# kahrendt/microWakeWord

Measured on NVIDIA H100. Metric: streams_x_frames_per_sec, higher is better.
Workload: dtype f32

## Files before the change

microwakeword_b200/csrc/mww_common.h:

```cpp
#pragma once

#include <stdint.h>

#if defined(__CUDACC__)
#define MWW_HD __host__ __device__ __forceinline__
#define MWW_D __device__ __forceinline__
#else
#define MWW_HD inline
#define MWW_D inline
#endif

namespace mww {

constexpr int kNumChannels = 40;
constexpr int kWindow = 480;
constexpr int kHop = 160;
constexpr int kFftSize = 512;
constexpr int kNcfft = 256;
constexpr float kFeatureScale = 0.0390625f;

MWW_HD int msb32(uint32_t x) {
#if defined(__CUDA_ARCH__)
    return 32 - __clz((int)x);
#else
    return x ? 32 - __builtin_clz(x) : 0;
#endif
}

MWW_HD int32_t sext16(int32_t v) { return (int32_t)(int16_t)v; }

MWW_HD uint32_t pack16(int32_t lo, int32_t hi) { return ((uint32_t)lo & 0xFFFFu) | ((uint32_t)hi << 16); }
MWW_HD int32_t unpack_lo(uint32_t w) { return (int32_t)(int16_t)(w & 0xFFFFu); }
MWW_HD int32_t unpack_hi(uint32_t w) { return ((int32_t)w) >> 16; }

MWW_HD int32_t max3i(int32_t a, int32_t b, int32_t c) { const int32_t m = a > b ? a : b; return m > c ? m : c; }
MWW_HD int32_t min3i(int32_t a, int32_t b, int32_t c) { const int32_t m = a < b ? a : b; return m < c ? m : c; }

MWW_HD int64_t mad_wide_s32(int32_t a, int32_t b, int64_t c) { return (int64_t)a * (int64_t)b + c; }

}
```

microwakeword_b200/csrc/mww_frontend.cu:

```cuda
#include <cuda_runtime.h>
#include <stdlib.h>

#include "mww_frontend_dev.cuh"
#include "mww_kernels.h"

namespace mww {

__device__ __forceinline__ void cp_async16(void *smem_dst, const void *gmem_src) {
    const unsigned dst = (unsigned)__cvta_generic_to_shared(smem_dst);
    asm volatile("cp.async.cg.shared.global [%0], [%1], 16;" ::"r"(dst), "l"(gmem_src));
}
__device__ __forceinline__ void cp_async_commit_and_wait_all() {
    asm volatile("cp.async.commit_group;\ncp.async.wait_group 0;" ::: "memory");
}

__device__ __forceinline__ void stage8(int16_t *dst, const int16_t *src) { cp_async16(dst, src); }
__device__ __forceinline__ void stage8(int16_t *dst, const float *src) {
    const float4 a = reinterpret_cast<const float4 *>(src)[0], b = reinterpret_cast<const float4 *>(src)[1];
    *reinterpret_cast<uint4 *>(dst) = make_uint4(pack16(pcm16_from_f32(a.x), pcm16_from_f32(a.y)), pack16(pcm16_from_f32(a.z), pcm16_from_f32(a.w)),
                                                 pack16(pcm16_from_f32(b.x), pcm16_from_f32(b.y)), pack16(pcm16_from_f32(b.z), pcm16_from_f32(b.w)));
}

template <typename T>
__device__ __forceinline__ void k1_load_audio_async(int tid, K1Smem &sm, int buf, const int16_t *carry, int used,
                                                    const T *audio, int n_samples, int f0) {
    const int base = kHop * f0;
    for (int v = tid; v < kGroupSamples / 8; v += kK1Threads) {
        const int vi = base + 8 * v;
        int16_t *dst = &sm.audio[buf][8 * v];
        if (vi < used) cp_async16(dst, carry + vi);
        else if (vi - used < n_samples) stage8(dst, audio + (vi - used));
        else *reinterpret_cast<uint4 *>(dst) = make_uint4(0, 0, 0, 0);
    }
}

template <typename T>
__device__ __forceinline__ void k1_packed_load_audio_async(int tid, K1Smem &sm, const int16_t *carry, int used, const T *audio,
                                                           long long audio_stride, int n_samples, long long s0, int n_streams, int spc, int fps) {
    const int span8 = (fps + 2) * (kHop / 8), used8 = used / 8, n8 = n_samples / 8;
    int16_t *dst0 = &sm.audio[0][0];
    for (int i = tid; i < spc * span8; i += kK1Threads) {
        const int sl = i / span8, v8 = i - sl * span8;
        int16_t *dst = dst0 + 8 * i;
        const long long s = s0 + sl;
        if (s < n_streams && v8 < used8) cp_async16(dst, carry + s * kWindow + 8 * v8);
        else if (s < n_streams && v8 - used8 < n8) stage8(dst, audio + s * audio_stride + 8 * (v8 - used8));
        else *reinterpret_cast<uint4 *>(dst) = make_uint4(0, 0, 0, 0);
    }
}

template <bool kFuseK2, int kOcc, typename T>
__global__ void __launch_bounds__(kK1Threads, kOcc)
k1_spectral_kernel(FrontendParams P, const int16_t *__restrict__ carry, int used,
                   const T *__restrict__ audio, long long audio_stride, int n_samples, int n_frames,
                   int groups_per_block, int vec_ok, uint32_t *__restrict__ vout, uint32_t *__restrict__ estimate,
                   uint16_t *__restrict__ feat, long long feat_stream_stride) {
    extern __shared__ __align__(16) unsigned char k1_smem_raw[];
    K1Smem &sm = *reinterpret_cast<K1Smem *>(k1_smem_raw);
    const int tid = threadIdx.x;
    const long long s = blockIdx.x;
    K1Lane lane;
    if (kOcc <= 3) k1_lane_init(tid, P, lane);
    else k1_stage_lane_twiddles(tid, sm, P);
    const K1LaneShared lane_sh{&sm.lane_tw[tid & 15][0]};
    k1_stage_tables(tid, sm, P);

    const int n_groups = (n_frames + kFramesPerGroup - 1) / kFramesPerGroup;
    const int g_begin = blockIdx.y * groups_per_block;
    const int g_end = min(g_begin + groups_per_block, n_groups);
    const int16_t *my_carry = carry + s * kWindow;
    const T *my_audio = audio + s * audio_stride;
    uint32_t est = 0;
    if (kFuseK2 && tid < kNumChannels) est = estimate[s * kNumChannels + tid];
    if (g_begin < g_end) {
        if (vec_ok) k1_load_audio_async(tid, sm, 0, my_carry, used, my_audio, n_samples, g_begin * kFramesPerGroup);
        else k1_load_audio(tid, sm, 0, my_carry, used, my_audio, n_samples, g_begin * kFramesPerGroup);
    }
    for (int g = g_begin; g < g_end; ++g) {
        const int buf = (g - g_begin) & 1;
        cp_async_commit_and_wait_all();
        __syncthreads();
        if (g + 1 < g_end) {
            if (vec_ok) k1_load_audio_async(tid, sm, buf ^ 1, my_carry, used, my_audio, n_samples, (g + 1) * kFramesPerGroup);
            else k1_load_audio(tid, sm, buf ^ 1, my_carry, used, my_audio, n_samples, (g + 1) * kFramesPerGroup);
        }
        const int f0 = g * kFramesPerGroup;
        K1Pass1Ctx ctx;
        k1_window_fft1<2>(tid, sm, buf, (kHop / 2) * (tid >> 4), P, ctx);
        __syncthreads();
        if (kOcc <= 3) k1_fft_pass2(tid, sm, lane); else k1_fft_pass2(tid, sm, lane_sh);
        __syncthreads();
        k1_real_energy(tid, sm, P);
        __syncthreads();
        const int f = f0 + (tid >> 4);
        if (!kFuseK2) {
            k1_filterbank(tid, sm, P, f < n_frames ? vout + (s * n_frames + f) * kNumChannels : nullptr);
        } else {
            k1_filterbank(tid, sm, P, &sm.A[tid >> 4][0]);
            __syncthreads();
            const int n_valid = min(kFramesPerGroup, n_frames - f0);
            if (tid < kNumChannels) k2_group_chain(tid, sm, n_valid, est);
            __syncthreads();
            k2_group_outputs(tid, sm, n_valid, feat + s * feat_stream_stride + (long long)f0 * kNumChannels);
        }
    }
    if (kFuseK2 && tid < kNumChannels) estimate[s * kNumChannels + tid] = est;
}

template <typename T>
__global__ void __launch_bounds__(kK1Threads, 3)
k1_spectral_hop_kernel(FrontendParams P, const int16_t *__restrict__ carry, int used, const T *__restrict__ audio,
                       long long audio_stride, int n_samples, int n_frames, int hop, uint32_t *__restrict__ estimate,
                       uint16_t *__restrict__ feat, long long feat_stream_stride) {
    extern __shared__ __align__(16) unsigned char k1_smem_raw[];
    K1Smem &sm = *reinterpret_cast<K1Smem *>(k1_smem_raw);
    const int tid = threadIdx.x;
    const long long s = blockIdx.x;
    K1Lane lane;
    k1_lane_init(tid, P, lane);
    k1_stage_tables(tid, sm, P);
    const int fpg = k1_hop_frames_per_group(hop);
    const int n_groups = (n_frames + fpg - 1) / fpg;
    const int16_t *my_carry = carry + s * kWindow;
    const T *my_audio = audio + s * audio_stride;
    uint32_t est = 0;
    if (tid < kNumChannels) est = estimate[s * kNumChannels + tid];
    for (int g = 0; g < n_groups; ++g) {
        const int f0 = g * fpg;
        __syncthreads();
        k1_hop_load_audio(tid, sm, my_carry, used, my_audio, n_samples, hop * f0, (fpg - 1) * hop + kWindow);
        __syncthreads();
        K1Pass1Ctx ctx;
        k1_window_fft1<2>(tid, sm, 0, k1_hop_pair_base(tid >> 4, hop, fpg), P, ctx);
        __syncthreads();
        k1_fft_pass2(tid, sm, lane);
        __syncthreads();
        k1_real_energy(tid, sm, P);
        __syncthreads();
        k1_filterbank(tid, sm, P, &sm.A[tid >> 4][0]);
        __syncthreads();
        const int n_valid = min(fpg, n_frames - f0);
        if (tid < kNumChannels) k2_group_chain(tid, sm, n_valid, est);
        __syncthreads();
        k2_group_outputs(tid, sm, n_valid, feat + s * feat_stream_stride + (long long)f0 * kNumChannels);
    }
    if (tid < kNumChannels) estimate[s * kNumChannels + tid] = est;
}

template <typename T>
__global__ void __launch_bounds__(kK1Threads, 3)
k1_spectral_packed_kernel(FrontendParams P, const int16_t *__restrict__ carry, int used,
                          const T *__restrict__ audio, long long audio_stride, int n_samples, int n_streams, int fps, int spc,
                          int vec_ok, uint32_t *__restrict__ vout) {
    extern __shared__ __align__(16) unsigned char k1_smem_raw[];
    K1Smem &sm = *reinterpret_cast<K1Smem *>(k1_smem_raw);
    const int tid = threadIdx.x;
    const long long s0 = (long long)blockIdx.x * spc;
    K1Lane lane;
    k1_lane_init(tid, P, lane);
    k1_stage_tables(tid, sm, P);
    if (vec_ok) {
        k1_packed_load_audio_async(tid, sm, carry, used, audio, audio_stride, n_samples, s0, n_streams, spc, fps);
        cp_async_commit_and_wait_all();
    } else {
        k1_packed_load_audio(tid, sm, carry, used, audio, audio_stride, n_samples, s0, n_streams, spc, fps);
    }
    __syncthreads();
    const int fl = tid >> 4;
    K1Pass1Ctx ctx;
    k1_window_fft1<2>(tid, sm, 0, k1_packed_pair_base(fl < spc * fps ? fl : 0, fps), P, ctx);
    __syncthreads();
    k1_fft_pass2(tid, sm, lane);
    __syncthreads();
    k1_real_energy(tid, sm, P);
    __syncthreads();
    const long long s = s0 + fl / fps;
    const bool active = fl < spc * fps && s < n_streams;
    k1_filterbank(tid, sm, P, active ? vout + (s * fps + fl % fps) * kNumChannels : nullptr);
}

template <typename T>
__global__ void __launch_bounds__(kK1Threads, 3)
k1k2_packed_kernel(FrontendParams P, int16_t *__restrict__ carry, int used, const T *__restrict__ audio,
                   long long audio_stride, int n_samples, int n_streams, int fps, int spc, int vec_ok, uint32_t *__restrict__ estimate,
                   uint16_t *__restrict__ feat, long long feat_stream_stride, int new_used) {
    extern __shared__ __align__(16) unsigned char k1_smem_raw[];
    K1Smem &sm = *reinterpret_cast<K1Smem *>(k1_smem_raw);
    const int tid = threadIdx.x;
    const long long s0 = (long long)blockIdx.x * spc;
    K1Lane lane;
    k1_lane_init(tid, P, lane);
    k1_stage_tables(tid, sm, P);
    if (vec_ok) {
        k1_packed_load_audio_async(tid, sm, carry, used, audio, audio_stride, n_samples, s0, n_streams, spc, fps);
        cp_async_commit_and_wait_all();
    } else {
        k1_packed_load_audio(tid, sm, carry, used, audio, audio_stride, n_samples, s0, n_streams, spc, fps);
    }
    __syncthreads();
    const int fl = tid >> 4;
    K1Pass1Ctx ctx;
    k1_window_fft1<2>(tid, sm, 0, k1_packed_pair_base(fl < spc * fps ? fl : 0, fps), P, ctx);
    __syncthreads();
    k1_fft_pass2(tid, sm, lane);
    __syncthreads();
    k1_real_energy(tid, sm, P);
    __syncthreads();
    k1_filterbank(tid, sm, P, fl < spc * fps ? &sm.A[fl][0] : nullptr);
    __syncthreads();
    for (int t = tid; t < spc * kNumChannels; t += kK1Threads) {
        const int sl = t / kNumChannels, ch = t - sl * kNumChannels;
        const long long s = s0 + sl;
        if (s < n_streams) {
            const uint32_t smoothing = (ch & 1) ? kOddSmoothing : kEvenSmoothing;
            uint32_t est = estimate[s * kNumChannels + ch];
            uint16_t *out = feat + s * feat_stream_stride + ch;
            for (int f = 0; f < fps; ++f) out[(long long)f * kNumChannels] = k2_channel_step(sm.A[sl * fps + f][ch], est, smoothing, sm.gain_lut, sm.log_lut);
            estimate[s * kNumChannels + ch] = est;
        }
    }
    const int span = (fps + 2) * kHop, consumed = fps * kHop;
    const int16_t *staged = &sm.audio[0][0];
    if (vec_ok) {
        for (int i = tid; i < spc * (kWindow / 8); i += kK1Threads) {
            const int sl = i / (kWindow / 8), v8 = i - sl * (kWindow / 8);
            if (s0 + sl >= n_streams) continue;
            uint4 v = make_uint4(0, 0, 0, 0);
            if (8 * v8 < new_used) v = *reinterpret_cast<const uint4 *>(staged + sl * span + consumed + 8 * v8);
            *reinterpret_cast<uint4 *>(carry + (s0 + sl) * kWindow + 8 * v8) = v;
        }
    } else {
        for (int i = tid; i < spc * kWindow; i += kK1Threads) {
            const int sl = i / kWindow, k = i - sl * kWindow;
            if (s0 + sl >= n_streams) continue;
            carry[(s0 + sl) * kWindow + k] = k < new_used ? staged[sl * span + consumed + k] : (int16_t)0;
        }
    }
}

__global__ void __launch_bounds__(256)
k2_temporal_kernel(FrontendParams P, const uint32_t *__restrict__ vin, int n_streams, int n_frames,
                   uint32_t *__restrict__ estimate, uint16_t *__restrict__ feat, long long feat_stream_stride) {
    __shared__ int16_t gain_lut[128];
    __shared__ uint16_t log_lut[132];
    for (int i = threadIdx.x; i < 128; i += blockDim.x) gain_lut[i] = P.gain_lut[i];
    for (int i = threadIdx.x; i < 132; i += blockDim.x) log_lut[i] = P.log_lut[i];
    __syncthreads();
    const long long idx = (long long)blockIdx.x * blockDim.x + threadIdx.x;
    if (idx >= (long long)n_streams * kNumChannels) return;
    const long long s = idx / kNumChannels;
    const int ch = (int)(idx - s * kNumChannels);
    const uint32_t smoothing = (ch & 1) ? kOddSmoothing : kEvenSmoothing;
    uint32_t est = estimate[idx];
    const uint32_t *v = vin + s * (long long)n_frames * kNumChannels + ch;
    uint16_t *out = feat + s * feat_stream_stride + ch;
    int f = 0;
    for (; f + 4 <= n_frames; f += 4) {
        uint32_t x[4];
#pragma unroll
        for (int q = 0; q < 4; ++q) x[q] = __ldcs(v + (long long)(f + q) * kNumChannels);
#pragma unroll
        for (int q = 0; q < 4; ++q) out[(long long)(f + q) * kNumChannels] = k2_channel_step(x[q], est, smoothing, gain_lut, log_lut);
    }
    for (; f < n_frames; ++f) out[(long long)f * kNumChannels] = k2_channel_step(v[(long long)f * kNumChannels], est, smoothing, gain_lut, log_lut);
    estimate[idx] = est;
}

template <typename T>
__global__ void __launch_bounds__(128)
carry_update_kernel(int16_t *__restrict__ carry, int used, const T *__restrict__ audio, long long audio_stride,
                    int n_samples, int consumed, int new_used) {
    const long long s = blockIdx.x;
    int16_t *c = carry + s * kWindow;
    const T *a = audio + s * audio_stride;
    int16_t tmp[4];
#pragma unroll
    for (int q = 0; q < 4; ++q) {
        const int i = threadIdx.x + 128 * q;
        int16_t val = 0;
        if (i < new_used) {
            const int vi = consumed + i;
            val = vi < used ? c[vi] : pcm16(a[vi - used]);
        }
        tmp[q] = val;
    }
    __syncthreads();
#pragma unroll
    for (int q = 0; q < 4; ++q) {
        const int i = threadIdx.x + 128 * q;
        if (i < kWindow) c[i] = tmp[q];
    }
}


namespace {
template <typename K>
cudaError_t k1_opt_in(K kernel, bool (&done)[64]) {
    if (!first_launch_on_this_device(done)) return cudaSuccess;
    return cudaFuncSetAttribute(kernel, cudaFuncAttributeMaxDynamicSharedMemorySize, kK1SmemBytes);
}
template <typename T>
int audio_vec_ok(const int16_t *carry, int used, const T *audio, long long audio_stride, int n_samples) {
    return (used % 8 == 0) && (n_samples % 8 == 0) && (audio_stride % 8 == 0) &&
           (reinterpret_cast<uintptr_t>(audio) % 16 == 0) && (reinterpret_cast<uintptr_t>(carry) % 16 == 0);
}
}

bool frontend_clip_fuses(int n_streams, int n_frames, int sm_count) {
    return n_frames > 8 && (long long)n_streams >= (long long)sm_count * 3 * 4;
}

template <typename T>
cudaError_t launch_k1(const FrontendParams &P, const int16_t *carry, int used, const T *audio,
                      long long audio_stride, int n_samples, int n_streams, int n_frames, uint32_t *vout, int sm_count,
                      cudaStream_t st) {
    if (n_frames <= 0 || n_streams <= 0) return cudaSuccess;
    const int vec_ok = audio_vec_ok(carry, used, audio, audio_stride, n_samples);
    if (n_frames <= 8 && n_streams >= 2) {
        static bool done[64] = {};
        cudaError_t e = k1_opt_in(k1_spectral_packed_kernel<T>, done);
        if (e != cudaSuccess) return e;
        const int spc = k1_packed_streams(n_frames);
        const unsigned grid = (unsigned)((n_streams + spc - 1) / spc);
        k1_spectral_packed_kernel<T><<<grid, kK1Threads, kK1SmemBytes, st>>>(P, carry, used, audio, audio_stride, n_samples, n_streams, n_frames, spc, vec_ok, vout);
        return cudaGetLastError();
    }
    static bool done[64] = {};
    cudaError_t e = k1_opt_in(k1_spectral_kernel<false, 3, T>, done);
    if (e != cudaSuccess) return e;
    const int n_groups = (n_frames + kFramesPerGroup - 1) / kFramesPerGroup;
    int chunks = 1;
    const long long want = (long long)sm_count * 3 * 4;
    if (n_streams < want) chunks = (int)min((long long)n_groups, (want + n_streams - 1) / n_streams);
    const int gpb = (n_groups + chunks - 1) / chunks;
    chunks = (n_groups + gpb - 1) / gpb;
    dim3 grid((unsigned)n_streams, (unsigned)chunks);
    k1_spectral_kernel<false, 3, T><<<grid, kK1Threads, kK1SmemBytes, st>>>(P, carry, used, audio, audio_stride, n_samples, n_frames, gpb, vec_ok, vout,
                                                                         nullptr, nullptr, 0);
    return cudaGetLastError();
}

template <typename T>
cudaError_t launch_frontend_clip_fused(const FrontendParams &P, const int16_t *carry, int used, const T *audio, long long audio_stride,
                                       int n_samples, int n_streams, int n_frames, uint32_t *estimate, uint16_t *feat, long long feat_stream_stride,
                                       cudaStream_t st) {
    if (n_frames <= 0 || n_streams <= 0) return cudaSuccess;
    static bool done3[64] = {}, done4[64] = {};
    static const int occ = getenv("MWW_K1_OCC") ? atoi(getenv("MWW_K1_OCC")) : 4;
    cudaError_t e = occ == 3 ? k1_opt_in(k1_spectral_kernel<true, 3, T>, done3) : k1_opt_in(k1_spectral_kernel<true, 4, T>, done4);
    if (e != cudaSuccess) return e;
    const int vec_ok = audio_vec_ok(carry, used, audio, audio_stride, n_samples);
    const int n_groups = (n_frames + kFramesPerGroup - 1) / kFramesPerGroup;
    dim3 grid((unsigned)n_streams, 1u);
    if (occ == 3)
        k1_spectral_kernel<true, 3, T><<<grid, kK1Threads, kK1SmemBytes, st>>>(P, carry, used, audio, audio_stride, n_samples, n_frames, n_groups, vec_ok,
                                                                               nullptr, estimate, feat, feat_stream_stride);
    else
        k1_spectral_kernel<true, 4, T><<<grid, kK1Threads, kK1SmemBytes, st>>>(P, carry, used, audio, audio_stride, n_samples, n_frames, n_groups, vec_ok,
                                                                               nullptr, estimate, feat, feat_stream_stride);
    return cudaGetLastError();
}

template <typename T>
cudaError_t launch_frontend_hop(const FrontendParams &P, const int16_t *carry, int used, const T *audio, long long audio_stride,
                                int n_samples, int n_streams, int n_frames, int hop, uint32_t *estimate, uint16_t *feat,
                                long long feat_stream_stride, cudaStream_t st) {
    if (n_frames <= 0 || n_streams <= 0) return cudaSuccess;
    static bool done[64] = {};
    cudaError_t e = k1_opt_in(k1_spectral_hop_kernel<T>, done);
    if (e != cudaSuccess) return e;
    k1_spectral_hop_kernel<T><<<(unsigned)n_streams, kK1Threads, kK1SmemBytes, st>>>(P, carry, used, audio, audio_stride, n_samples, n_frames, hop,
                                                                                    estimate, feat, feat_stream_stride);
    return cudaGetLastError();
}

bool frontend_fusable(int used, int n_samples, int n_frames) {
    const int new_used = used + n_samples - n_frames * kHop;
    return n_frames >= 1 && n_frames <= 8 && new_used >= 0 && new_used <= 2 * kHop;
}

template <typename T>
cudaError_t launch_frontend_fused(const FrontendParams &P, int16_t *carry, int used, const T *audio,
                                  long long audio_stride, int n_samples, int n_streams, int n_frames, uint32_t *estimate, uint16_t *feat,
                                  long long feat_stream_stride, cudaStream_t st) {
    if (n_streams <= 0) return cudaSuccess;
    static bool done[64] = {};
    cudaError_t e = k1_opt_in(k1k2_packed_kernel<T>, done);
    if (e != cudaSuccess) return e;
    const int vec_ok = audio_vec_ok(carry, used, audio, audio_stride, n_samples);
    const int spc = k1_packed_streams(n_frames);
    const unsigned grid = (unsigned)((n_streams + spc - 1) / spc);
    k1k2_packed_kernel<T><<<grid, kK1Threads, kK1SmemBytes, st>>>(P, carry, used, audio, audio_stride, n_samples, n_streams, n_frames, spc, vec_ok,
                                                                  estimate, feat, feat_stream_stride, used + n_samples - n_frames * kHop);
    return cudaGetLastError();
}

cudaError_t launch_k2(const FrontendParams &P, const uint32_t *vin, int n_streams, int n_frames, uint32_t *estimate,
                      uint16_t *feat, long long feat_stream_stride, cudaStream_t st) {
    if (n_frames <= 0 || n_streams <= 0) return cudaSuccess;
    const long long total = (long long)n_streams * kNumChannels;
    const unsigned blocks = (unsigned)((total + 255) / 256);
    k2_temporal_kernel<<<blocks, 256, 0, st>>>(P, vin, n_streams, n_frames, estimate, feat, feat_stream_stride);
    return cudaGetLastError();
}

template <typename T>
cudaError_t launch_carry_update(int16_t *carry, int used, const T *audio, long long audio_stride, int n_samples,
                                int n_streams, int consumed, int new_used, cudaStream_t st) {
    if (n_streams <= 0) return cudaSuccess;
    carry_update_kernel<T><<<(unsigned)n_streams, 128, 0, st>>>(carry, used, audio, audio_stride, n_samples, consumed, new_used);
    return cudaGetLastError();
}

#define MWW_FRONTEND_INSTANTIATE(T)                                                                                            \
    template cudaError_t launch_k1<T>(const FrontendParams &, const int16_t *, int, const T *, long long, int, int, int, uint32_t *, \
                                      int, cudaStream_t);                                                                      \
    template cudaError_t launch_frontend_clip_fused<T>(const FrontendParams &, const int16_t *, int, const T *, long long, int, int, \
                                                       int, uint32_t *, uint16_t *, long long, cudaStream_t);                 \
    template cudaError_t launch_frontend_hop<T>(const FrontendParams &, const int16_t *, int, const T *, long long, int, int, int, \
                                                int, uint32_t *, uint16_t *, long long, cudaStream_t);                        \
    template cudaError_t launch_frontend_fused<T>(const FrontendParams &, int16_t *, int, const T *, long long, int, int, int,   \
                                                  uint32_t *, uint16_t *, long long, cudaStream_t);                           \
    template cudaError_t launch_carry_update<T>(int16_t *, int, const T *, long long, int, int, int, int, cudaStream_t);
MWW_FRONTEND_INSTANTIATE(int16_t)
MWW_FRONTEND_INSTANTIATE(float)
#undef MWW_FRONTEND_INSTANTIATE

}
```

microwakeword_b200/csrc/mww_frontend_dev.cuh:

```cuda
#pragma once

#include "mww_common.h"
#include "mww_tables.h"

#if !defined(__CUDA_ARCH__)
#include <math.h>
#endif

namespace mww {

constexpr int kFramesPerGroup = 16;
constexpr int kK1Threads = 256;
constexpr int kRowWords = 272;
constexpr int kGroupSamples = (kFramesPerGroup + 2) * kHop;


struct K1Smem {
    uint32_t A[kFramesPerGroup][kRowWords];
    uint32_t B[kFramesPerGroup][kRowWords];
    int16_t audio[2][kGroupSamples];
    uint16_t lane_max[kFramesPerGroup][16];
    int32_t shift[kFramesPerGroup];
    int32_t fb_coef[kFbCoefWords];
    int16_t gain_lut[128];
    uint16_t log_lut[132];
    uint32_t lane_tw[16][15];
};
constexpr int kK1SmemBytes = (int)sizeof(K1Smem);

MWW_HD void k1_stage_tables(int tid, K1Smem &sm, const FrontendParams &P) {
    for (int i = tid; i < kFbCoefWords; i += kK1Threads) sm.fb_coef[i] = P.fb_coef[i];
    for (int i = tid; i < 128; i += kK1Threads) sm.gain_lut[i] = P.gain_lut[i];
    for (int i = tid; i < 132; i += kK1Threads) sm.log_lut[i] = P.log_lut[i];
}

struct K1Lane {
    int32_t t3r[3], t3i[3];
    int32_t t4r[12], t4i[12];
};

struct K1LaneShared { const uint32_t *row; };


MWW_HD int32_t fixdiv4(int32_t x) { return (x * 8191 + 16384) >> 15; }
MWW_HD int32_t fixdiv2(int32_t x) { return (x * 16383 + 16384) >> 15; }

MWW_HD void cmul_q15(int32_t ar, int32_t ai, int32_t wr, int32_t wi, int32_t &mr, int32_t &mi) {
    mr = (ar * wr - ai * wi + 16384) >> 15;
    mi = (ar * wi + ai * wr + 16384) >> 15;
}

MWW_HD void bfly4_core(int32_t &r0, int32_t &i0, int32_t &r1, int32_t &i1, int32_t &r2, int32_t &i2, int32_t &r3, int32_t &i3) {
    const int32_t s5r = r0 - r2, s5i = i0 - i2;
    const int32_t f0r = r0 + r2, f0i = i0 + i2;
    const int32_t s3r = r1 + r3, s3i = i1 + i3;
    const int32_t s4r = r1 - r3, s4i = i1 - i3;
    r2 = f0r - s3r; i2 = f0i - s3i;
    r0 = f0r + s3r; i0 = f0i + s3i;
    r1 = s5r + s4i; i1 = s5i - s4r;
    r3 = s5r - s4i; i3 = s5i + s4r;
}


MWW_HD uint64_t sq32(uint32_t r) { return (uint64_t)r * r; }

MWW_HD uint32_t isqrt64_round(uint64_t x) {
#if defined(__CUDA_ARCH__)
    const float xf = __ull2float_rn(x);
    const float rs = rsqrtf(xf);
    uint32_t r = __float2uint_rz(xf * rs);
    const int64_t d = (int64_t)(x - sq32(r));
    const int64_t r1 = (int64_t)r + (int64_t)__float2int_rd(__ll2float_rn(d) * (0.5f * rs));
#else
    const float xf = (float)x;
    const float rs = x ? 1.0f / sqrtf(xf) : 0.0f;
    const float rf = xf * rs;
    uint32_t r = rf >= 4294967040.0f ? 0xFFFFFFFFu : (uint32_t)rf;
    const int64_t d = (int64_t)(x - sq32(r));
    const int64_t r1 = (int64_t)r + (int64_t)floorf((float)d * (0.5f * rs));
#endif
    r = r1 > 0xFFFFFFFFll ? 0xFFFFFFFFu : (r1 < 0 ? 0u : (uint32_t)r1);
#pragma unroll
    for (int pass = 0; pass < 2; ++pass) r -= (sq32(r) > x) ? 1u : 0u;
    uint64_t rem = x - sq32(r);
#pragma unroll
    for (int pass = 0; pass < 2; ++pass) {
        const bool up = rem > 2ull * r;
        rem -= up ? 2ull * r + 1 : 0ull;
        r += up ? 1u : 0u;
    }
    const uint32_t cap = (x >> 32) == 0 ? 0xFFFFu : 0xFFFFFFFFu;
    r += (rem > r && r < cap) ? 1u : 0u;
    r = r > cap ? cap : r;
    return x == 0 ? 0u : r;
}

MWW_HD uint32_t isqrt64_round_fast(uint64_t x) {
    if (x >> 48) return isqrt64_round(x);
#if defined(__CUDA_ARCH__)
    const uint32_t r = __double2uint_rz(sqrt(__ull2double_rn(x)) + 0.5);
#else
    const uint32_t r = (uint32_t)(sqrt((double)x) + 0.5);
#endif
    const uint32_t cap = (x >> 32) == 0 ? 0xFFFFu : 0xFFFFFFFFu;
    return r > cap ? cap : r;
}


MWW_HD void k1_lane_init(int tid, const FrontendParams &P, K1Lane &L) {
    const int b = tid & 15;
    for (int j = 0; j < 3; ++j) {
        const uint32_t w = P.tw[4 * b * (j + 1)];
        L.t3r[j] = unpack_lo(w); L.t3i[j] = unpack_hi(w);
    }
    for (int j = 0; j < 4; ++j) {
        const int kp = 16 * j + b;
        for (int q = 0; q < 3; ++q) {
            const uint32_t w = P.tw[kp * (q + 1)];
            L.t4r[3 * j + q] = unpack_lo(w); L.t4i[3 * j + q] = unpack_hi(w);
        }
    }
}

MWW_HD void k1_stage_lane_twiddles(int tid, K1Smem &sm, const FrontendParams &P) {
    for (int i = tid; i < 16 * 15; i += kK1Threads) {
        const int b = i / 15, e = i - 15 * b;
        int idx;
        if (e < 3) idx = 4 * b * (e + 1);
        else { const int j = (e - 3) / 3, q = (e - 3) - 3 * j; idx = (16 * j + b) * (q + 1); }
        sm.lane_tw[b][e] = P.tw[idx];
    }
}
MWW_HD void lane_tw3(const K1Lane &L, int q, int32_t &wr, int32_t &wi) { wr = L.t3r[q]; wi = L.t3i[q]; }
MWW_HD void lane_tw4(const K1Lane &L, int i, int32_t &wr, int32_t &wi) { wr = L.t4r[i]; wi = L.t4i[i]; }
MWW_HD void lane_tw3(const K1LaneShared &L, int q, int32_t &wr, int32_t &wi) { const uint32_t w = L.row[q]; wr = unpack_lo(w); wi = unpack_hi(w); }
MWW_HD void lane_tw4(const K1LaneShared &L, int i, int32_t &wr, int32_t &wi) { const uint32_t w = L.row[3 + i]; wr = unpack_lo(w); wi = unpack_hi(w); }

MWW_HD int16_t pcm16_from_f32(float x) {
    const float y = x * 32768.0f;
    if (y != y) return 0;
    const float c = y < -32768.0f ? -32768.0f : (y > 32767.0f ? 32767.0f : y);
    return (int16_t)(int32_t)c;
}
MWW_HD int16_t pcm16(int16_t v) { return v; }
MWW_HD int16_t pcm16(float v) { return pcm16_from_f32(v); }

template <typename T>
MWW_HD void k1_load_audio(int tid, K1Smem &sm, int buf, const int16_t *carry, int used, const T *audio, int n_samples, int f0) {
    const int base = kHop * f0;
    for (int i = tid; i < kGroupSamples; i += kK1Threads) {
        const int vi = base + i;
        int16_t s = 0;
        if (vi < used) s = carry[vi];
        else if (vi - used < n_samples) s = pcm16(audio[vi - used]);
        sm.audio[buf][i] = s;
    }
}

MWW_HD int k1_hop_frames_per_group(int hop) {
    const int by_span = (2 * kGroupSamples - kWindow) / hop + 1;
    return by_span < kFramesPerGroup ? by_span : kFramesPerGroup;
}
template <typename T>
MWW_HD void k1_hop_load_audio(int tid, K1Smem &sm, const int16_t *carry, int used, const T *audio, int n_samples, int base, int span) {
    int16_t *dst = &sm.audio[0][0];
    for (int i = tid; i < span; i += kK1Threads) {
        const int vi = base + i;
        int16_t s = 0;
        if (vi < used) s = carry[vi];
        else if (vi - used < n_samples) s = pcm16(audio[vi - used]);
        dst[i] = s;
    }
}
MWW_HD int k1_hop_pair_base(int fl, int hop, int fpg) { return (hop / 2) * (fl < fpg ? fl : fpg - 1); }

struct K1Pass1Ctx { int32_t xr[16], xi[16]; };

template <int PART>
MWW_HD void k1_window_fft1(int tid, K1Smem &sm, int buf, int pair_base, const FrontendParams &P, K1Pass1Ctx &ctx) {
    const int fl = tid >> 4, a = tid & 15;
    const int c = (a >> 2) + 4 * (a & 3);
    int32_t (&xr)[16] = ctx.xr;
    int32_t (&xi)[16] = ctx.xi;
    if (PART != 1) {
        const uint32_t *pairs = reinterpret_cast<const uint32_t *>(sm.audio[buf]) + pair_base;
        int32_t mx = 0, mn = 0;
#pragma unroll
        for (int b = 0; b < 16; ++b) {
            const int j = (b >> 2) + 4 * (b & 3);
            if (j == 15) { xr[b] = 0; xi[b] = 0; continue; }
            const int p = c + 16 * j;
            const uint32_t sw = pairs[p];
            const uint32_t cw = P.win_pairs[p];
            const int32_t v0 = (unpack_lo(sw) * unpack_lo(cw)) >> 12;
            const int32_t v1 = (unpack_hi(sw) * unpack_hi(cw)) >> 12;
            xr[b] = v0; xi[b] = v1;
            if (j == 7) {
                const int32_t m0 = v0 == -32768 ? 0 : v0, m1 = v1 == -32768 ? 0 : v1;
                mx = max3i(mx, m0, m1); mn = min3i(mn, m0, m1);
            } else {
                mx = max3i(mx, v0, v1); mn = min3i(mn, v0, v1);
            }
        }
        const int32_t m = mx > -mn ? mx : -mn;
        sm.lane_max[fl][a] = (uint16_t)m;
    }
#if defined(__CUDA_ARCH__)
    if (PART == 2) __syncwarp();
#endif
    if (PART == 0) return;
    int32_t mxa = 0;
#pragma unroll
    for (int i = 0; i < 16; ++i) { const int32_t v = sm.lane_max[fl][i]; mxa = v > mxa ? v : mxa; }
    const int shift = 15 - msb32((uint32_t)mxa);
    if (a == 0) sm.shift[fl] = shift;
    const int32_t k4 = 8191 << shift;
#pragma unroll
    for (int g = 0; g < 4; ++g) {
#pragma unroll
        for (int q = 0; q < 4; ++q) {
            const int b = 4 * g + q;
            const int j = (b >> 2) + 4 * (b & 3);
            if (j == 7) {
                xr[b] = fixdiv4(sext16(xr[b] << shift)); xi[b] = fixdiv4(sext16(xi[b] << shift));
            } else {
                xr[b] = (xr[b] * k4 + 16384) >> 15; xi[b] = (xi[b] * k4 + 16384) >> 15;
            }
        }
        bfly4_core(xr[4 * g], xi[4 * g], xr[4 * g + 1], xi[4 * g + 1], xr[4 * g + 2], xi[4 * g + 2], xr[4 * g + 3], xi[4 * g + 3]);
    }
#pragma unroll
    for (int k = 0; k < 4; ++k) {
#pragma unroll
        for (int q = 0; q < 4; ++q) { xr[k + 4 * q] = fixdiv4(xr[k + 4 * q]); xi[k + 4 * q] = fixdiv4(xi[k + 4 * q]); }
        if (k > 0) {
#pragma unroll
            for (int q = 1; q < 4; ++q) {
                int32_t mr, mi;
                cmul_q15(xr[k + 4 * q], xi[k + 4 * q], P.tw2[(k - 1) * 3 + (q - 1)][0], P.tw2[(k - 1) * 3 + (q - 1)][1], mr, mi);
                xr[k + 4 * q] = mr; xi[k + 4 * q] = mi;
            }
        }
        bfly4_core(xr[k], xi[k], xr[k + 4], xi[k + 4], xr[k + 8], xi[k + 8], xr[k + 12], xi[k + 12]);
    }
#pragma unroll
    for (int b = 0; b < 16; ++b) sm.B[fl][17 * a + b] = pack16(xr[b], xi[b]);
}

MWW_HD int k1_packed_streams(int fps) {
    const int by_slots = kFramesPerGroup / fps;
    const int by_smem = (2 * kGroupSamples) / ((fps + 2) * kHop);
    return by_slots < by_smem ? by_slots : by_smem;
}
template <typename T>
MWW_HD void k1_packed_load_audio(int tid, K1Smem &sm, const int16_t *carry, int used, const T *audio, long long audio_stride,
                                 int n_samples, long long s0, int n_streams, int spc, int fps) {
    const int span = (fps + 2) * kHop;
    int16_t *dst = &sm.audio[0][0];
    for (int i = tid; i < spc * span; i += kK1Threads) {
        const int sl = i / span, vi = i - sl * span;
        int16_t v = 0;
        if (s0 + sl < n_streams) {
            if (vi < used) v = carry[(s0 + sl) * kWindow + vi];
            else if (vi - used < n_samples) v = pcm16(audio[(s0 + sl) * audio_stride + (vi - used)]);
        }
        dst[i] = v;
    }
}
MWW_HD int k1_packed_pair_base(int fl, int fps) { return (fl / fps) * ((fps + 2) * (kHop / 2)) + (kHop / 2) * (fl % fps); }

template <typename LaneT>
MWW_HD void k1_fft_pass2(int tid, K1Smem &sm, const LaneT &L) {
    const int fl = tid >> 4, b = tid & 15;
    int32_t yr[16], yi[16];
#pragma unroll
    for (int a = 0; a < 16; ++a) {
        const uint32_t w = sm.B[fl][17 * a + b];
        yr[a] = unpack_lo(w); yi[a] = unpack_hi(w);
    }
#pragma unroll
    for (int c = 0; c < 4; ++c) {
#pragma unroll
        for (int q = 0; q < 4; ++q) { yr[4 * c + q] = fixdiv4(yr[4 * c + q]); yi[4 * c + q] = fixdiv4(yi[4 * c + q]); }
#pragma unroll
        for (int q = 1; q < 4; ++q) {
            int32_t mr, mi, wr, wi;
            lane_tw3(L, q - 1, wr, wi);
            cmul_q15(yr[4 * c + q], yi[4 * c + q], wr, wi, mr, mi);
            yr[4 * c + q] = mr; yi[4 * c + q] = mi;
        }
        bfly4_core(yr[4 * c], yi[4 * c], yr[4 * c + 1], yi[4 * c + 1], yr[4 * c + 2], yi[4 * c + 2], yr[4 * c + 3], yi[4 * c + 3]);
    }
#pragma unroll
    for (int j = 0; j < 4; ++j) {
#pragma unroll
        for (int q = 0; q < 4; ++q) { yr[4 * q + j] = fixdiv4(sext16(yr[4 * q + j])); yi[4 * q + j] = fixdiv4(sext16(yi[4 * q + j])); }
#pragma unroll
        for (int q = 1; q < 4; ++q) {
            int32_t mr, mi, wr, wi;
            lane_tw4(L, 3 * j + q - 1, wr, wi);
            cmul_q15(yr[4 * q + j], yi[4 * q + j], wr, wi, mr, mi);
            yr[4 * q + j] = mr; yi[4 * q + j] = mi;
        }
        bfly4_core(yr[j], yi[j], yr[4 + j], yi[4 + j], yr[8 + j], yi[8 + j], yr[12 + j], yi[12 + j]);
    }
#pragma unroll
    for (int a = 0; a < 16; ++a) sm.A[fl][b + 16 * a] = pack16(yr[a], yi[a]);
}

MWW_HD void k1_real_energy(int tid, K1Smem &sm, const FrontendParams &P) {
    const int fl = tid >> 4, l = tid & 15;
    if (l == 0) { sm.B[fl][0] = 0; sm.B[fl][kEnergyOffset] = 0; }
#pragma unroll
    for (int t = 0; t < 8; ++t) {
        const int k = 1 + 16 * t + l;
        const uint32_t wk = sm.A[fl][k];
        const uint32_t wn = sm.A[fl][kNcfft - k];
        const uint32_t ws = P.super_tw[k - 1];
        const int32_t pr = fixdiv2(unpack_lo(wk)), pi = fixdiv2(unpack_hi(wk));
        const int32_t nr = fixdiv2(unpack_lo(wn)), ni = fixdiv2(sext16(-unpack_hi(wn)));
        const int32_t f1r = pr + nr, f1i = pi + ni;
        const int32_t f2r = pr - nr, f2i = pi - ni;
        int32_t tr, ti;
        cmul_q15(f2r, f2i, unpack_lo(ws), unpack_hi(ws), tr, ti);
        tr = sext16(tr); ti = sext16(ti);
        const int32_t ar = sext16((f1r + tr) >> 1), ai = sext16((f1i + ti) >> 1);
        const int32_t br = sext16((f1r - tr) >> 1), bi = sext16((ti - f1i) >> 1);
        sm.B[fl][k + kEnergyOffset] = (uint32_t)(ar * ar) + (uint32_t)(ai * ai);
        sm.B[fl][kNcfft - k + kEnergyOffset] = (uint32_t)(br * br) + (uint32_t)(bi * bi);
    }
}

struct Pair32 { uint32_t x, y; };
MWW_HD Pair32 load_pair(const uint32_t *p) {
#if defined(__CUDA_ARCH__)
    const uint2 v = *reinterpret_cast<const uint2 *>(p);
    return Pair32{v.x, v.y};
#else
    return Pair32{p[0], p[1]};
#endif
}
MWW_HD void k1_filterbank(int tid, K1Smem &sm, const FrontendParams &P, uint32_t *vout_frame ) {
    const int fl = tid >> 4, l = tid & 15;
    const int sh = sm.shift[fl];
#pragma unroll
    for (int s = 0; s < kFbSlots; ++s) {
        if (fb_len(s) == 0) continue;
        const FbSlot slot = P.fb_slots[l * kFbSlots + s];
        int64_t acc = 0;
        const uint32_t *e = &sm.B[fl][slot.word0];
        const uint32_t *cf = reinterpret_cast<const uint32_t *>(&sm.fb_coef[slot.coef_off]);
#pragma unroll
        for (int j = 0; j < fb_len(s) / 2; ++j) {
            const Pair32 ev = load_pair(e + 2 * j), cv = load_pair(cf + 2 * j);
            acc = mad_wide_s32((int32_t)ev.x, (int32_t)cv.x, acc);
            acc = mad_wide_s32((int32_t)ev.y, (int32_t)cv.y, acc);
        }
        if (slot.ch >= 0 && vout_frame) vout_frame[slot.ch] = isqrt64_round_fast((uint64_t)acc) >> sh;
    }
}


MWW_HD int32_t wide_dynamic_function(uint32_t x, const int16_t *lut) {
    if (x <= 2) return lut[x];
    const int interval = msb32(x);
    const int16_t *p = lut + 4 * interval - 6;
    const int32_t frac = (int32_t)(((interval < 11) ? (x << (11 - interval)) : (x >> (interval - 11))) & 0x3FF);
    int32_t r = ((int32_t)p[2] * frac) >> 5;
    r += (int32_t)((uint32_t)(int32_t)p[1] << 5);
    r *= frac;
    r = (r + (1 << 14)) >> 15;
    r += p[0];
    return (int32_t)(int16_t)r;
}

MWW_HD uint32_t pcan_shrink(uint32_t x) {
    if (x < (2u << 12)) return (x * x) >> 20;
    return (x >> 6) - 64u;
}

MWW_HD uint32_t log_scale(uint32_t x, const uint16_t *lut) {
    const uint32_t integer = (uint32_t)msb32(x) - 1;
    int32_t frac = (int32_t)(x - (1u << integer));
    if (integer < 16) frac <<= (16 - integer); else frac >>= (integer - 16);
    const uint32_t seg = (uint32_t)frac >> 9;
    const int32_t c0 = lut[seg], c1 = lut[seg + 1];
    const int32_t rel = ((c1 - c0) * (frac - (int32_t)(seg << 9))) >> 16;
    const uint32_t log2v = (integer << 16) + (uint32_t)(frac + c0 + rel);
    const uint32_t loge = (uint32_t)((45426ull * log2v + 32768u) >> 16);
    return ((loge << kLogScaleShift) + 32768u) >> 16;
}

MWW_HD uint32_t k2_estimate_update(uint32_t v, uint32_t est, uint32_t smoothing) {
    const uint32_t scaled = v << kSmoothingBits;
    return (uint32_t)((((uint64_t)scaled * smoothing) + ((uint64_t)est * ((1u << kNoiseBits) - smoothing))) >> kNoiseBits);
}

MWW_HD uint16_t k2_output(uint32_t v, uint32_t est, const int16_t *gain_lut, const uint16_t *log_lut) {
    const uint32_t scaled = v << kSmoothingBits;
    const uint32_t e = est > scaled ? scaled : est;
    const uint32_t fl = (uint32_t)(((uint64_t)v * kMinSignalRemaining) >> kNoiseBits);
    const uint32_t sub = (scaled - e) >> kSmoothingBits;
    uint32_t sig = sub > fl ? sub : fl;
    const uint32_t gain = (uint32_t)wide_dynamic_function(est, gain_lut);
    const uint32_t snr = (uint32_t)(((uint64_t)sig * gain) >> kPcanSnrShift);
    sig = pcan_shrink(snr);
    sig <<= kLogCorrectionBits;
    sig = sig > 1 ? log_scale(sig, log_lut) : 0;
    return (uint16_t)(sig < 0xFFFFu ? sig : 0xFFFFu);
}

MWW_HD uint16_t k2_channel_step(uint32_t v, uint32_t &est, uint32_t smoothing, const int16_t *gain_lut, const uint16_t *log_lut) {
    est = k2_estimate_update(v, est, smoothing);
    return k2_output(v, est, gain_lut, log_lut);
}

MWW_HD void k2_group_chain(int ch, K1Smem &sm, int n_valid, uint32_t &est) {
    const uint32_t smoothing = (ch & 1) ? kOddSmoothing : kEvenSmoothing;
    for (int f = 0; f < n_valid; ++f) {
        est = k2_estimate_update(sm.A[f][ch], est, smoothing);
        sm.B[f][ch] = est;
    }
}
MWW_HD void k2_group_outputs(int tid, K1Smem &sm, int n_valid, uint16_t *feat_group ) {
    for (int i = tid; i < n_valid * kNumChannels; i += kK1Threads) {
        const int f = i / kNumChannels, ch = i - f * kNumChannels;
        feat_group[i] = k2_output(sm.A[f][ch], sm.B[f][ch], sm.gain_lut, sm.log_lut);
    }
}

}
```

Before: 454.1 million.

## Cap registers, pre-unpack tables into shared memory, and branchless fixed-point helpers

Replaces the launch bounds with a 72-register cap and static-asserts that shared memory fits four CTAs per SM, aiming at higher occupancy. The window and super-twiddle tables are pre-unpacked into Int2 entries in shared memory instead of being read from params, and the window multiply uses mulhi with a pre-shifted coefficient. The lane-max reduction becomes vectorized u16x2 max, and the log and gain helpers use clz and funnel shifts in place of branches. The filterbank takes a fast double-sqrt path with a warp-wide fallback when any accumulator exceeds 48 bits. The register cap risks spills, and the bit-trick rewrites risk subtle numeric mismatches.

```diff
diff --git a/microwakeword_b200/csrc/mww_common.h b/microwakeword_b200/csrc/mww_common.h
--- a/microwakeword_b200/csrc/mww_common.h
+++ b/microwakeword_b200/csrc/mww_common.h
@@ -19,13 +19,44 @@
 constexpr int kNcfft = 256;
 constexpr float kFeatureScale = 0.0390625f;
 
-MWW_HD int msb32(uint32_t x) {
+MWW_HD int clz32(uint32_t x) {
 #if defined(__CUDA_ARCH__)
-    return 32 - __clz((int)x);
+    return __clz((int)x);
 #else
-    return x ? 32 - __builtin_clz(x) : 0;
+    return x ? __builtin_clz(x) : 32;
 #endif
 }
+
+MWW_HD int msb32(uint32_t x) { return 32 - clz32(x); }
+
+
+MWW_HD uint32_t shl_clamp32(uint32_t x, int s) {
+#if defined(__CUDA_ARCH__)
+    return __funnelshift_lc(0u, x, (unsigned)s);
+#else
+    return (uint32_t)((uint64_t)x << s);
+#endif
+}
+
+MWW_HD int32_t mulhi_s32(int32_t a, int32_t b) {
+#if defined(__CUDA_ARCH__)
+    return __mulhi(a, b);
+#else
+    return (int32_t)(((int64_t)a * (int64_t)b) >> 32);
+#endif
+}
+
+MWW_HD uint32_t vmax_u16x2(uint32_t a, uint32_t b) {
+#if defined(__CUDA_ARCH__)
+    return __vmaxu2(a, b);
+#else
+    const uint32_t lo = (a & 0xFFFFu) > (b & 0xFFFFu) ? (a & 0xFFFFu) : (b & 0xFFFFu);
+    const uint32_t hi = (a >> 16) > (b >> 16) ? (a >> 16) : (b >> 16);
+    return lo | (hi << 16);
+#endif
+}
+
+struct alignas(8) Int2 { int32_t x, y; };
 
 MWW_HD int32_t sext16(int32_t v) { return (int32_t)(int16_t)v; }
 
diff --git a/microwakeword_b200/csrc/mww_frontend.cu b/microwakeword_b200/csrc/mww_frontend.cu
--- a/microwakeword_b200/csrc/mww_frontend.cu
+++ b/microwakeword_b200/csrc/mww_frontend.cu
@@ -108,7 +108,7 @@
 }
 
 template <typename T>
-__global__ void __launch_bounds__(kK1Threads, 3)
+__global__ void __maxnreg__(72)
 k1_spectral_hop_kernel(FrontendParams P, const int16_t *__restrict__ carry, int used, const T *__restrict__ audio,
                        long long audio_stride, int n_samples, int n_frames, int hop, uint32_t *__restrict__ estimate,
                        uint16_t *__restrict__ feat, long long feat_stream_stride) {
diff --git a/microwakeword_b200/csrc/mww_frontend_dev.cuh b/microwakeword_b200/csrc/mww_frontend_dev.cuh
--- a/microwakeword_b200/csrc/mww_frontend_dev.cuh
+++ b/microwakeword_b200/csrc/mww_frontend_dev.cuh
@@ -1,4 +1,6 @@
 #pragma once
+
+#include <stddef.h>
 
 #include "mww_common.h"
 #include "mww_tables.h"
@@ -18,20 +20,26 @@
 struct K1Smem {
     uint32_t A[kFramesPerGroup][kRowWords];
     uint32_t B[kFramesPerGroup][kRowWords];
+    Int2 win16[240];
+    Int2 super_tw[128];
+    Int2 lane_tw[16][15];
     int16_t audio[2][kGroupSamples];
     uint16_t lane_max[kFramesPerGroup][16];
     int32_t shift[kFramesPerGroup];
     int32_t fb_coef[kFbCoefWords];
     int16_t gain_lut[128];
     uint16_t log_lut[132];
-    uint32_t lane_tw[16][15];
 };
 constexpr int kK1SmemBytes = (int)sizeof(K1Smem);
+static_assert(4 * (sizeof(K1Smem) + 1024) <= 228 * 1024, "K1Smem: four CTAs per SM");
+static_assert(offsetof(K1Smem, audio) % 16 == 0 && offsetof(K1Smem, lane_max) % 16 == 0, "K1Smem: 16-byte staging and lane_max rows");
 
 MWW_HD void k1_stage_tables(int tid, K1Smem &sm, const FrontendParams &P) {
     for (int i = tid; i < kFbCoefWords; i += kK1Threads) sm.fb_coef[i] = P.fb_coef[i];
     for (int i = tid; i < 128; i += kK1Threads) sm.gain_lut[i] = P.gain_lut[i];
     for (int i = tid; i < 132; i += kK1Threads) sm.log_lut[i] = P.log_lut[i];
+    for (int i = tid; i < 240; i += kK1Threads) { const uint32_t w = P.win_pairs[i]; sm.win16[i] = Int2{unpack_lo(w) << 4, unpack_hi(w) << 4}; }
+    for (int i = tid; i < 128; i += kK1Threads) { const uint32_t w = P.super_tw[i]; sm.super_tw[i] = Int2{unpack_lo(w), unpack_hi(w)}; }
 }
 
 struct K1Lane {
@@ -39,7 +47,7 @@
     int32_t t4r[12], t4i[12];
 };
 
-struct K1LaneShared { const uint32_t *row; };
+struct K1LaneShared { const Int2 *row; };
 
 
 MWW_HD int32_t fixdiv4(int32_t x) { return (x * 8191 + 16384) >> 15; }
@@ -95,8 +103,7 @@
     return x == 0 ? 0u : r;
 }
 
-MWW_HD uint32_t isqrt64_round_fast(uint64_t x) {
-    if (x >> 48) return isqrt64_round(x);
+MWW_HD uint32_t isqrt64_round_below48(uint64_t x) {
 #if defined(__CUDA_ARCH__)
     const uint32_t r = __double2uint_rz(sqrt(__ull2double_rn(x)) + 0.5);
 #else
@@ -105,6 +112,7 @@
     const uint32_t cap = (x >> 32) == 0 ? 0xFFFFu : 0xFFFFFFFFu;
     return r > cap ? cap : r;
 }
+MWW_HD uint32_t isqrt64_round_fast(uint64_t x) { return (x >> 48) ? isqrt64_round(x) : isqrt64_round_below48(x); }
 
 
 MWW_HD void k1_lane_init(int tid, const FrontendParams &P, K1Lane &L) {
@@ -128,13 +136,14 @@
         int idx;
         if (e < 3) idx = 4 * b * (e + 1);
         else { const int j = (e - 3) / 3, q = (e - 3) - 3 * j; idx = (16 * j + b) * (q + 1); }
-        sm.lane_tw[b][e] = P.tw[idx];
+        const uint32_t w = P.tw[idx];
+        sm.lane_tw[b][e] = Int2{unpack_lo(w), unpack_hi(w)};
     }
 }
 MWW_HD void lane_tw3(const K1Lane &L, int q, int32_t &wr, int32_t &wi) { wr = L.t3r[q]; wi = L.t3i[q]; }
 MWW_HD void lane_tw4(const K1Lane &L, int i, int32_t &wr, int32_t &wi) { wr = L.t4r[i]; wi = L.t4i[i]; }
-MWW_HD void lane_tw3(const K1LaneShared &L, int q, int32_t &wr, int32_t &wi) { const uint32_t w = L.row[q]; wr = unpack_lo(w); wi = unpack_hi(w); }
-MWW_HD void lane_tw4(const K1LaneShared &L, int i, int32_t &wr, int32_t &wi) { const uint32_t w = L.row[3 + i]; wr = unpack_lo(w); wi = unpack_hi(w); }
+MWW_HD void lane_tw3(const K1LaneShared &L, int q, int32_t &wr, int32_t &wi) { const Int2 w = L.row[q]; wr = w.x; wi = w.y; }
+MWW_HD void lane_tw4(const K1LaneShared &L, int i, int32_t &wr, int32_t &wi) { const Int2 w = L.row[3 + i]; wr = w.x; wi = w.y; }
 
 MWW_HD int16_t pcm16_from_f32(float x) {
     const float y = x * 32768.0f;
@@ -191,9 +200,9 @@
             if (j == 15) { xr[b] = 0; xi[b] = 0; continue; }
             const int p = c + 16 * j;
             const uint32_t sw = pairs[p];
-            const uint32_t cw = P.win_pairs[p];
-            const int32_t v0 = (unpack_lo(sw) * unpack_lo(cw)) >> 12;
-            const int32_t v1 = (unpack_hi(sw) * unpack_hi(cw)) >> 12;
+            const Int2 cw = sm.win16[p];
+            const int32_t v0 = mulhi_s32((int32_t)(sw << 16), cw.x);
+            const int32_t v1 = mulhi_s32((int32_t)(sw & 0xFFFF0000u), cw.y);
             xr[b] = v0; xi[b] = v1;
             if (j == 7) {
                 const int32_t m0 = v0 == -32768 ? 0 : v0, m1 = v1 == -32768 ? 0 : v1;
@@ -209,10 +218,20 @@
     if (PART == 2) __syncwarp();
 #endif
     if (PART == 0) return;
-    int32_t mxa = 0;
-#pragma unroll
-    for (int i = 0; i < 16; ++i) { const int32_t v = sm.lane_max[fl][i]; mxa = v > mxa ? v : mxa; }
-    const int shift = 15 - msb32((uint32_t)mxa);
+    uint32_t m2 = 0;
+#pragma unroll
+    for (int h = 0; h < 2; ++h) {
+        uint32_t q[4];
+#if defined(__CUDA_ARCH__)
+        const uint4 v = reinterpret_cast<const uint4 *>(sm.lane_max[fl])[h];
+        q[0] = v.x; q[1] = v.y; q[2] = v.z; q[3] = v.w;
+#else
+        for (int i = 0; i < 4; ++i) q[i] = (uint32_t)sm.lane_max[fl][8 * h + 2 * i] | ((uint32_t)sm.lane_max[fl][8 * h + 2 * i + 1] << 16);
+#endif
+        m2 = vmax_u16x2(m2, vmax_u16x2(vmax_u16x2(q[0], q[1]), vmax_u16x2(q[2], q[3])));
+    }
+    const uint32_t mxa = (m2 & 0xFFFFu) > (m2 >> 16) ? (m2 & 0xFFFFu) : (m2 >> 16);
+    const int shift = 15 - msb32(mxa);
     if (a == 0) sm.shift[fl] = shift;
     const int32_t k4 = 8191 << shift;
 #pragma unroll
@@ -316,16 +335,16 @@
         const int k = 1 + 16 * t + l;
         const uint32_t wk = sm.A[fl][k];
         const uint32_t wn = sm.A[fl][kNcfft - k];
-        const uint32_t ws = P.super_tw[k - 1];
+        const Int2 ws = sm.super_tw[k - 1];
         const int32_t pr = fixdiv2(unpack_lo(wk)), pi = fixdiv2(unpack_hi(wk));
         const int32_t nr = fixdiv2(unpack_lo(wn)), ni = fixdiv2(sext16(-unpack_hi(wn)));
         const int32_t f1r = pr + nr, f1i = pi + ni;
         const int32_t f2r = pr - nr, f2i = pi - ni;
         int32_t tr, ti;
-        cmul_q15(f2r, f2i, unpack_lo(ws), unpack_hi(ws), tr, ti);
+        cmul_q15(f2r, f2i, ws.x, ws.y, tr, ti);
         tr = sext16(tr); ti = sext16(ti);
-        const int32_t ar = sext16((f1r + tr) >> 1), ai = sext16((f1i + ti) >> 1);
-        const int32_t br = sext16((f1r - tr) >> 1), bi = sext16((ti - f1i) >> 1);
+        const int32_t ar = (f1r + tr) >> 1, ai = (f1i + ti) >> 1;
+        const int32_t br = (f1r - tr) >> 1, bi = (ti - f1i) >> 1;
         sm.B[fl][k + kEnergyOffset] = (uint32_t)(ar * ar) + (uint32_t)(ai * ai);
         sm.B[fl][kNcfft - k + kEnergyOffset] = (uint32_t)(br * br) + (uint32_t)(bi * bi);
     }
@@ -340,32 +359,46 @@
     return Pair32{p[0], p[1]};
 #endif
 }
+MWW_HD int64_t k1_fb_accumulate(const K1Smem &sm, int fl, const FbSlot &slot, int len) {
+    int64_t acc = 0;
+    const uint32_t *e = &sm.B[fl][slot.word0];
+    const uint32_t *cf = reinterpret_cast<const uint32_t *>(&sm.fb_coef[slot.coef_off]);
+#pragma unroll
+    for (int j = 0; j < len / 2; ++j) {
+        const Pair32 ev = load_pair(e + 2 * j), cv = load_pair(cf + 2 * j);
+        acc = mad_wide_s32((int32_t)ev.x, (int32_t)cv.x, acc);
+        acc = mad_wide_s32((int32_t)ev.y, (int32_t)cv.y, acc);
+    }
+    return acc;
+}
 MWW_HD void k1_filterbank(int tid, K1Smem &sm, const FrontendParams &P, uint32_t *vout_frame ) {
     const int fl = tid >> 4, l = tid & 15;
     const int sh = sm.shift[fl];
+    bool big = false;
 #pragma unroll
     for (int s = 0; s < kFbSlots; ++s) {
         if (fb_len(s) == 0) continue;
         const FbSlot slot = P.fb_slots[l * kFbSlots + s];
-        int64_t acc = 0;
-        const uint32_t *e = &sm.B[fl][slot.word0];
-        const uint32_t *cf = reinterpret_cast<const uint32_t *>(&sm.fb_coef[slot.coef_off]);
-#pragma unroll
-        for (int j = 0; j < fb_len(s) / 2; ++j) {
-            const Pair32 ev = load_pair(e + 2 * j), cv = load_pair(cf + 2 * j);
-            acc = mad_wide_s32((int32_t)ev.x, (int32_t)cv.x, acc);
-            acc = mad_wide_s32((int32_t)ev.y, (int32_t)cv.y, acc);
-        }
-        if (slot.ch >= 0 && vout_frame) vout_frame[slot.ch] = isqrt64_round_fast((uint64_t)acc) >> sh;
+        const uint64_t acc = (uint64_t)k1_fb_accumulate(sm, fl, slot, fb_len(s));
+        big |= (acc >> 48) != 0;
+        if (slot.ch >= 0 && vout_frame) vout_frame[slot.ch] = isqrt64_round_below48(acc & 0xFFFFFFFFFFFFull) >> sh;
+    }
+#if defined(__CUDA_ARCH__)
+    big = __any_sync(0xFFFFFFFFu, big);
+#endif
+    if (!big || !vout_frame) return;
+    for (int s = 0; s < kFbSlots; ++s) {
+        if (fb_len(s) == 0) continue;
+        const FbSlot slot = P.fb_slots[l * kFbSlots + s];
+        if (slot.ch >= 0) vout_frame[slot.ch] = isqrt64_round_fast((uint64_t)k1_fb_accumulate(sm, fl, slot, fb_len(s))) >> sh;
     }
 }
 
 
 MWW_HD int32_t wide_dynamic_function(uint32_t x, const int16_t *lut) {
-    if (x <= 2) return lut[x];
-    const int interval = msb32(x);
-    const int16_t *p = lut + 4 * interval - 6;
-    const int32_t frac = (int32_t)(((interval < 11) ? (x << (11 - interval)) : (x >> (interval - 11))) & 0x3FF);
+    const int lz = clz32(x);
+    const int16_t *p = lut + (x <= 2 ? (int)x : 122 - 4 * lz);
+    const int32_t frac = (int32_t)((shl_clamp32(x, lz) >> 21) & 0x3FF);
     int32_t r = ((int32_t)p[2] * frac) >> 5;
     r += (int32_t)((uint32_t)(int32_t)p[1] << 5);
     r *= frac;
@@ -375,14 +408,14 @@
 }
 
 MWW_HD uint32_t pcan_shrink(uint32_t x) {
-    if (x < (2u << 12)) return (x * x) >> 20;
-    return (x >> 6) - 64u;
+    const uint32_t quad = (x * x) >> 20, lin = (x >> 6) - 64u;
+    return x < (2u << 12) ? quad : lin;
 }
 
 MWW_HD uint32_t log_scale(uint32_t x, const uint16_t *lut) {
-    const uint32_t integer = (uint32_t)msb32(x) - 1;
-    int32_t frac = (int32_t)(x - (1u << integer));
-    if (integer < 16) frac <<= (16 - integer); else frac >>= (integer - 16);
+    const int lz = clz32(x);
+    const uint32_t integer = 31u - (uint32_t)lz;
+    const int32_t frac = (int32_t)(shl_clamp32(x, lz + 1) >> 16);
     const uint32_t seg = (uint32_t)frac >> 9;
     const int32_t c0 = lut[seg], c1 = lut[seg + 1];
     const int32_t rel = ((c1 - c0) * (frac - (int32_t)(seg << 9))) >> 16;
@@ -406,7 +439,8 @@
     const uint32_t snr = (uint32_t)(((uint64_t)sig * gain) >> kPcanSnrShift);
     sig = pcan_shrink(snr);
     sig <<= kLogCorrectionBits;
-    sig = sig > 1 ? log_scale(sig, log_lut) : 0;
+    const uint32_t lg = log_scale(sig, log_lut);
+    sig = sig > 1 ? lg : 0;
     return (uint16_t)(sig < 0xFFFFu ? sig : 0xFFFFu);
 }
 
```

New measurement: 480.0 million, median of 6. 1.06x the previous value.
